# Ren-Okubo/diffusion_model

Hardware: AMD Instinct MI355X
Metric: atoms*denoise-steps/sec, 64-atom SiO2 T=1000 (higher is better)
Workload: dtype bf16; 1 GPU; 64-atom SiO2 cells x 256 graphs/GPU, 4-layer EGNN (H=36, W=1024, m=256), T=1000 reverse steps, fully connected (E=1032192/GPU); global_batch=256, parallelism=replicas x1 (no data-path collective)

## Files before the change

diffusion_model_amd/_lib.py:

```python
import ctypes as C
import os

_HERE = os.path.dirname(os.path.abspath(__file__))
LIB_PATH = os.environ.get("EGNN_LIB", os.path.join(_HERE, "libegnn_amd.so"))

PREC_F32, PREC_BF16, PREC_BF16X3, PREC_F16, PREC_F16C8 = 0, 1, 2, 3, 4
NORM_CALL, NORM_GRAPH = 0, 1
PRECISIONS = {"fp32": PREC_F32, "f32": PREC_F32, "float32": PREC_F32, "bf16": PREC_BF16, "bfloat16": PREC_BF16,
              "bf16x3": PREC_BF16X3, "f16c8": PREC_F16C8, "fp16": PREC_F16, "f16": PREC_F16, "float16": PREC_F16}
NORM_SCOPES = {"call": NORM_CALL, "graph": NORM_GRAPH}
OPTIM_ADAM, OPTIM_ADAMW_AMSGRAD, OPTIM_RADAM_SF = 0, 1, 2
KABSCH_CENTERS = {"centroid": 0, "first": 1}
KABSCH_FLIPS = {"row": 0, "column": 1}
ASSIGN_MAX_ATOMS = 1024
STRUCT_MAX_TYPES, STRUCT_MAX_ATOMS = 4, 32768
STRUCT_CENTRE_BLOCK, STRUCT_CHUNK, STRUCT_BOND_CENTRES = 64, 1024, 8
CELL_MAX_TYPES, CELL_MAX_SHELLS, CELL_MAX_ENV_ATOMS, CELL_SHIFT_CODES = 4, 4, 1024, 729
TOPO_MAX_ATOMS, TOPO_MAX_DEGREE, TOPO_BRANCH_MODULUS, TOPO_MAX_LENGTH = 1024, 32, 7, 64
RING_MAX_SITES, RING_MAX_SIZE = 4096, 32
SOAP_MAX_TYPES, SOAP_MAX_N, SOAP_MAX_L, SOAP_MAX_K = 4, 16, 10, 8
SQ_MAX_TYPES, SQ_MAX_Q, SQ_MAX_BINS, SQ_MAX_ATOMS, SQ_MAX_VECTORS = 4, 4096, 4096, 32768, 1 << 24
SQ_ROW_BLOCK, SQ_CHUNK, SQ_VECTOR_BLOCK = 64, 256, 256
SQ_WINDOWS = {None: 0, "none": 0, "lorch": 1}
CELL_CENTRE_BLOCK = 64
PREALIGN_MIN_ATOMS = 5


_FLAGS_FALLBACK = b"FLAGS := --offload-arch=gfx950 -O3 -std=c++17 -fPIC -ffp-contract=off -fno-slp-vectorize -fvisibility=hidden"


def _flags_line() -> bytes:
    try:
        with open(os.path.join(os.path.dirname(_HERE), "Makefile"), "rb") as f:
            flags = [l for l in f.read().splitlines() if l.startswith(b"FLAGS")]
        return b"\n".join(flags)
    except OSError:
        return _FLAGS_FALLBACK


def _sources_sha256(names) -> str:
    import hashlib
    h = hashlib.sha256()
    csrc = os.path.join(_HERE, "csrc")
    for name in names:
        with open(os.path.join(csrc, name), "rb") as f:
            h.update(name.encode() + b"\0" + f.read())
    h.update(_flags_line())
    return h.hexdigest()


def edge_kernel_sources_sha256() -> str:
    return _sources_sha256(("edge_x_m16.hip", "edge_bf16_v4.hip", "pack.hip", "edge_tile.h", "kernels.h", "common.h", "layer_pack.h",
                            "diag.h"))


def forward_sources_sha256() -> str:
    return _sources_sha256(("egnn_forward.hip", "host_logic.h", "host_logic.cpp", "pack.hip", "edge_x_m16.hip", "edge_bf16_v4.hip", "edge_bf16_v3.hip", "edge_small.hip",
                            "edge_bf16x3.hip", "edge_f16c8w.hip", "edge_f16c8w_mphase2.inc", "edge_f16c8w_mphasek.inc", "node_bf16.hip",
                            "edge_tile.h", "kernels.h", "common.h", "layer_pack.h", "diag.h"))


def training_sources_sha256() -> str:
    import glob
    import hashlib
    h = hashlib.sha256()
    csrc = os.path.join(_HERE, "csrc")
    names = sorted(glob.glob(os.path.join(csrc, "*.hip")) + glob.glob(os.path.join(csrc, "*.h")) + glob.glob(os.path.join(csrc, "*.cpp")) +
                   glob.glob(os.path.join(csrc, "*.inc")))
    names += [os.path.join(_HERE, "autograd.py"), os.path.join(_HERE, "gemm.py")]
    for path in names:
        with open(path, "rb") as f:
            h.update(os.path.basename(path).encode() + b"\0" + f.read())
    h.update(_flags_line())
    return h.hexdigest()


_vp, _i, _f, _u64 = C.c_void_p, C.c_int, C.c_float, C.c_uint64
_fp = C.POINTER(C.c_float)


class OptimConsts(C.Structure):
    _fields_ = [(name, C.c_float) for name in ("beta2", "one_minus_beta2", "eps", "weight_decay", "one_minus_beta1",
                                               "bias_correction2_sqrt", "step_size", "decay_mul", "bias_correction2", "ckp1",
                                               "adaptive_y_lr", "lr")] + [("rectified", C.c_int32)]


_pp, _i64p, _dp = C.POINTER(C.c_void_p), C.POINTER(C.c_int64), C.POINTER(C.c_double)

SIGNATURES = {
    "egnn_last_error": (C.c_char_p, []),
    "egnn_version": (_i, []),
    "egnn_create": (_i, [C.POINTER(_vp), _i]),
    "egnn_destroy": (_i, [_vp]),
    "egnn_set_model": (_i, [_vp] + [_i] * 6),
    "egnn_pack_layer": (_i, [_vp, _vp, _i] + [_vp] * 16),
    "egnn_set_graph": (_i, [_vp, _i, _i, _i] + [_vp] * 5),
    "egnn_set_side_stream": (_i, [_vp, _vp]),
    "egcl_forward": (_i, [_vp, _vp, _i, _i, _i] + [_vp] * 4),
    "egcl_forward_begin": (_i, [_vp, _vp, _i, _i, _i] + [_vp] * 3),
    "egcl_forward_end": (_i, [_vp, _vp, _i, _i, _i] + [_vp] * 5),
    "egnn_forward": (_i, [_vp, _vp, _i, _i] + [_vp] * 4),
    "egcl_read_aggregates": (_i, [_vp, _vp, _i] + [_vp] * 3),
    "egcl_backward_l1_act": (_i, [_vp, _i, _i, _i] + [_vp] * 7),
    "egcl_backward_heads": (_i, [_vp, _i, _i, _i, _i] + [_vp] * 20),
    "egcl_backward_l1_grad": (_i, [_vp, _i, _i, _i] + [_vp] * 7),
    "egcl_backward_gather_in": (_i, [_vp, _i, _i, _i, _i] + [_vp] * 6),
    "egcl_backward_scatter": (_i, [_vp, _i, _i, _i, _i] + [_vp] * 9),
    "egcl_backward_first_reduce": (_i, [_vp, _i, _i, _i, _i, _vp, _vp, _vp, _vp, _vp, _i, _vp, _i] + [_vp] * 9),
    "egcl_backward_node_act": (_i, [_vp, _i, _i, _vp, _i, _vp, _vp, _i, _vp, _vp, _i, _vp]),
    "egcl_backward_scatter_geom": (_i, [_vp, _i, _i] + [_vp] * 8),
    "egcl_backward_fused_supported": (_i, [_vp]),
    "egcl_backward_table": (_i, [_vp, _vp, _i, _vp]),
    "egcl_backward_edge_recompute": (_i, [_vp, _vp, _i, _vp, _vp, _vp, _i, _i] + [_vp] * 11),
    "egcl_backward_dgrad": (_i, [_vp, _vp, _i, _vp, _i, _i] + [_vp] * 4),
    "egcl_backward_dgrad_reduce": (_i, [_vp, _vp, _i, _vp, _i, _i] + [_vp] * 6),
    "egcl_forward_save": (_i, [_vp, _vp, _i, _i] + [_vp] * 9),
    "egcl_backward_heads_saved": (_i, [_vp, _vp, _i, _vp, _vp, _vp, _i, _i] + [_vp] * 10),
    "egnn_gemm_tn_workspace_bytes": (C.c_size_t, [_i, _i, _i]),
    "egnn_gemm_tn_bf16": (_i, [_vp, _i, _i, _i, _vp, _i, _vp, _i, _f, _vp, _i, _i, _i, _i, _vp, C.c_size_t]),
    "egnn_gemm_rows_pack": (_i, [_vp, _i, _i, _vp, _i, _vp]),
    "egnn_gemm_rows_bf16": (_i, [_vp, _i, _vp, _i, _i, _vp, _vp, _i, _i, _vp, _vp, _i, _i, _i]),
    "egnn_gamma_tilde": (_i, [_vp, _i, _i, _vp, _vp, _vp, _vp, _vp]),
    "egnn_dense_rows": (_i, [_vp, _i, _i, _i, _vp, _vp, _vp, _i, _vp]),
    "egnn_eps": (_i, [_vp, _i, _i, _i, _vp, _i] + [_vp] * 5),
    "egnn_remove_mean": (_i, [_vp, _i, _i, _vp, _i, _vp, _vp]),
    "schedule_table_build": (_i, [_i, C.c_double, C.c_double, _fp, _fp, _fp]),
    "schedule_table_from_alpha": (_i, [_i, _fp, _fp, _fp]),
    "ddpm_reverse_step": (_i, [_vp, _i, _i, _i, _vp, _i, _f, _f, _f, _vp, _i, _vp, _vp, _vp, _i]),
    "egnn_sampler_prepare": (_i, [_vp, _i, _i, _f, _vp, _vp, _u64]),
    "egnn_sampler_set_mode": (_i, [_vp, _i]),
    "egnn_sampler_init": (_i, [_vp, _vp, _vp, _vp]),
    "egnn_sampler_run": (_i, [_vp, _vp, _i, _i, _i, _i, _vp, _vp]),
    "egnn_sampler_final": (_i, [_vp, _vp, _i, _i] + [_vp] * 5),
    "egnn_sampler_state": (_i, [_vp, _vp, _vp, _vp, _vp, C.POINTER(_i)]),
    "ddpm_sampler_init": (_i, [_vp, _i, _i, _i, _i, _i, _vp, _vp, _f, _u64] + [_vp] * 6),
    "ddpm_sampler_step": (_i, [_vp, _i, _i, _i, _i, _i, _i, _vp, _vp, _f, _u64] + [_vp] * 7),
    "ddpm_sampler_final": (_i, [_vp, _i, _i, _i, _i, _i, _vp, _vp, _f, _u64] + [_vp] * 10),
    "egnn_fc_graph_build": (_i, [_vp, _i, _i] + [_vp] * 6),
    "egnn_radius_graph_count": (_i, [_vp, _i, _vp, _vp, _vp, _f, _vp]),
    "egnn_radius_graph_fill": (_i, [_vp, _i, _vp, _vp, _vp, _f, _vp, _vp, _vp]),
    "egnn_rdf": (_i, [_vp, _i, _vp, _vp, C.c_double, C.c_double, _f, _i, _i, _vp]),
    "egnn_si_o_si": (_i, [_vp, _i, _i, _vp, _vp, _vp, _f, _vp]),
    "egnn_kabsch": (_i, [_vp, _i, _vp, _vp, _vp, _i, _i, _vp, _vp, _i, _vp]),
    "egnn_kabsch_ordered": (_i, [_vp, _i, _vp, _vp, _vp, _vp, _i, _i, _vp]),
    "egnn_kabsch_backward": (_i, [_vp, _i, _vp, _vp, _vp, _vp, _i, _i, _vp, _vp, _vp]),
    "egnn_kabsch_grad_host": (_i, [_i, _dp, _dp, _i, _i, _dp, _dp, C.c_double, _dp, _dp]),
    "egnn_kabsch_perm_workspace_bytes": (C.c_size_t, [_i, _i]),
    "egnn_kabsch_perm": (_i, [_vp, _i, _vp, _vp, _vp, _i, _vp, _vp, _vp, _vp, _vp, C.c_size_t]),
    "egnn_assign": (_i, [_vp, _i, _vp, _vp, _vp, _i, _vp, _vp, _vp]),
    "egnn_assign_prealign": (_i, [_vp, _i, _vp, _vp, _vp, _i, _vp, _vp]),
    "egnn_struct_pair_counts": (_i, [_vp, _i, _i, _vp, _vp, _vp, _i, _vp, _i, C.c_double, _i, _vp]),
    "egnn_struct_bonds": (_i, [_vp, _i, _i, _vp, _vp, _vp, _i, _vp, _i, _f, C.c_double, _i, _vp, _vp, _vp]),
    "egnn_struct_rdf_finish": (_i, [_vp, _i, _i, _vp, _vp, _vp, C.c_double, C.c_double, C.c_double, _i, _vp]),
    "egnn_struct_counts_host": (_i, [_i, _i, _vp, _vp, _vp, C.c_double, _i, _f, C.c_double, _i, _vp, _vp, _vp, _vp]),
    "egnn_topo_bonds": (_i, [_vp, _i, _i, _i, _vp, _vp, _vp, _i, _vp, _vp, _vp, _vp, _vp]),
    "egnn_topo_paths": (_i, [_vp, _i, _i, _i, _vp, _vp, _i, _vp, _vp, _vp, _vp, _i, _vp, _vp, _vp, _vp, _vp]),
    "egnn_topo_tanimoto": (_i, [_vp, _i, _i, _vp, _i, _vp, _i, _vp, _vp, _vp, _vp]),
    "egnn_topo_host": (_i, [_i, _i, _vp, _vp, _vp, _vp, _i] + [_vp] * 8 + [_i] + [_vp] * 4),
    "egnn_rings": (_i, [_vp, _i, _vp, _i, _vp, _vp, _vp, _i, _i, _vp, _vp, _i, _i, _i] + [_vp] * 8),
    "egnn_rings_host": (_i, [_i, _vp, _i, _vp, _vp, _vp, _i, _i, _vp, _vp, _i, _i, _i] + [_vp] * 4),
    "egnn_soap_features": (_i, [_i, _i, _i]),
    "egnn_soap_table_doubles": (_i, [_i, _i]),
    "egnn_soap_descriptor": (_i, [_vp, _i, _i, _i, _vp, _vp, _vp, _i, _i, C.c_double, _vp, _i, _vp, _vp, _vp, _vp]),
    "egnn_soap_cosine": (_i, [_vp, _i, _i, _vp, _i, _vp, _i, _vp, _vp]),
    "egnn_soap_gram": (_i, [_vp, _i, _vp, _i, _vp, _i, _vp, _vp]),
    "egnn_spectrum_nearest": (_i, [_vp, _i, _i, _i, _i] + [_vp] * 6),
    "egnn_soap_host": (_i, [_i, _i, _i, _vp, _vp, _vp, _i, _i, C.c_double, _vp, _i, _vp, _vp, _vp, _i, _vp, _i, _vp, _i, _i, _vp, _vp, _vp,
                            _i, _i, _i, _i] + [_vp] * 6),
    "egnn_cell_bonds_count": (_i, [_vp, _i, _i, _vp, _vp, _vp, _vp, _vp, C.c_double, _vp, _i, _vp]),
    "egnn_cell_bonds_fill": (_i, [_vp, _i, _i, _vp, _vp, _vp, _vp, _vp, C.c_double, _vp, _i, _vp, _i, _vp, _vp]),
    "egnn_cell_env_count": (_i, [_vp, _i, _i, _vp, _vp, _vp, _i, _vp, _vp, _i, _vp, _vp, _i, _i, _vp]),
    "egnn_cell_env_fill": (_i, [_vp, _i, _i, _i, _vp, _vp, _vp, _vp, _vp, _vp, _vp, _i, _vp, _vp, _i, _vp, _vp, _i, _i, _vp, _i] + [_vp] * 4),
    "egnn_cell_env_host": (_i, [_i, _i, _vp, _vp, _vp, _vp, C.c_double, _i, _vp, _vp, _i, _i, _vp, C.c_int64, _vp, _vp, _vp, C.c_int64] + [_vp] * 4),
    "egnn_sq_debye": (_i, [_vp, _i, _i, _vp, _vp, _vp, _i, _i, _vp, _vp, C.c_double, _i, _vp, _i, _vp, _vp, _vp]),
    "egnn_sq_cell_plan": (_i, [_i, _vp, C.c_double, _vp, _vp]),
    "egnn_sq_cell_count": (_i, [_vp, _i, _vp, _vp, _vp, _vp, C.c_double, _i, _vp]),
    "egnn_sq_cell_rho": (_i, [_vp, _i, _i, _i] + [_vp] * 10 + [C.c_double, C.c_double, _i, _i, _vp, _i, _vp, _i] + [_vp] * 4),
    "egnn_sq_cell_shells": (_i, [_vp, _i, _i, _i, _vp, _vp, _i] + [_vp] * 6),
    "egnn_sq_host": (_i, [_i, _i, _i, _vp, _vp, _vp, _i, _vp, C.c_double, _i, _vp, _i, _i, _i, _vp, _vp, _vp, _vp, C.c_double, C.c_double, _i,
                          C.c_int64] + [_vp] * 8),
    "egnn_optim_step": (_i, [_vp, _i, _i, _pp, _pp, _pp, _pp, _pp, _i64p, C.POINTER(OptimConsts)]),
    "egnn_optim_interp": (_i, [_vp, _i, _pp, _pp, _i64p, _f]),
    "egnn_optim_tensors_per_launch": (_i, []),
    "egnn_debug_stamps": (_i, [_vp, C.POINTER(C.c_uint64)]),
    "egnn_profile_enable": (_i, [_vp, _i]),
    "egnn_profile_read": (_i, [_vp, _fp, C.POINTER(_i), _fp]),
}

_lib = None


def lib():
    global _lib
    if _lib is None:
        if not os.path.exists(LIB_PATH):
            raise RuntimeError(
                f"{LIB_PATH} not found: build the HIP extension first (`make` at the repo root or "
                "`python -c 'import __graft_entry__ as g; g.build()'`). There is no CPU fallback.")
        handle = C.CDLL(LIB_PATH)
        for name, (res, args) in SIGNATURES.items():
            fn = getattr(handle, name)
            fn.restype, fn.argtypes = res, args
        _lib = handle
    return _lib


class EgnnError(RuntimeError):
    pass


def check(rc):
    if rc != 0:
# ... 17 lines not shown
```

diffusion_model_amd/csrc/edge_x_m16.hip:

```cpp
#include <cstdlib>

#include "diag.h"
#include "edge_tile.h"

namespace egnn {

namespace {

#ifdef EGNN_EXP_WGSTAMP
__device__ unsigned long long g_xwg_stamps[20000][12];
#define WG_STAMP(k) DIAG_WG_STAMP(g_xwg_stamps, 20000, k)
#define WG_STAMP_HW() DIAG_WG_STAMP_HW(g_xwg_stamps, 20000, 5)
#else
#define WG_STAMP(k)
#define WG_STAMP_HW()
#endif

using namespace tile128;
constexpr size_t kA1 = (size_t)8 * kR * 16;
__host__ __device__ constexpr size_t x16_smem_bytes(int KP) { return kOffLoop + 2 * kA1 + (size_t)KP * 4; }
static_assert(x16_smem_bytes(256) == 48192 && x16_smem_bytes(512) == 49216 && x16_smem_bytes(1024) == 51264,
              "LDS allocation of the 16x16x32 coordinate kernels");

typedef __attribute__((ext_vector_type(4))) float f32x4v;

template <bool SAVE, typename V8 = bf16x8, bool PERSIST = false>
__global__ __launch_bounds__(kTileThreads, 2) void edge_x_m16_kernel(const EdgeParams p) {
  static_assert(!(SAVE && OpTraits<V8>::f16), "the training forward keeps bf16 activations");
  static_assert(!(SAVE && PERSIST), "the persistent form is the inference kernel");
  if constexpr (OpTraits<V8>::f16) f16_saturate_mode();
  extern __shared__ __attribute__((aligned(16))) char smem[];
  const Lds L(smem);
  char* s_a1 = smem + kOffLoop;
  float* s_wd = reinterpret_cast<float*>(s_a1 + 2 * kA1);

  const int tid = threadIdx.x, lane = tid & 63;
  const int wave = __builtin_amdgcn_readfirstlane(tid >> 6);
  const int r15 = lane & 15, q4 = lane >> 4;
  const int KP = p.WxP;
  const int nsplit = p.WxP / 512;
  const int NC = KP / kChunkK, KS = KP / 32;
  const rsrc_t rs_tab = make_rsrc(p.table, diag::drop_table_loads(p.dbg) ? 0u : (unsigned)((size_t)p.N * p.TC * 2));
  const rsrc_t rs_w = make_rsrc(p.w2x, diag::drop_weight_loads(p.dbg) ? 0u : (unsigned)((size_t)p.WxP * KP * 2));
  const unsigned offP = 0u, offQ = (unsigned)p.WxP * 2u;
  const unsigned lane16 = lane * 16u;
  const int nunits = PERSIST ? ((p.E + kR - 1) / kR) * nsplit : (int)gridDim.x;
  UnitH uc0, uc1;
  V8 bq[2][4];
  int pf_d0, pf_s0, pf_d1, pf_s1, pf_d, pf_s, pf_r0, pf_r1;
  float pf_x[6];
  auto unit_of = [&](const int bv, int& tile_o, int& half_o) {
    const int jj = xcd_tile(bv, nunits);
    tile_o = jj / nsplit;
    half_o = jj - tile_o * nsplit;
  };
  auto prefetch_indices = [&](const int bv, const int tq) {
    int t, h;
    unit_of(bv, t, h);
    const int ne0 = t * kR, nnv = min(kR, p.E - ne0), br = tq >> 3;
    const bool r0 = br < nnv, r1 = br + 64 < nnv, rt = tq < nnv && tq < kR;
    pf_d0 = r0 ? p.edge_dst[ne0 + br] : 0; pf_s0 = r0 ? p.edge_src[ne0 + br] : 0;
    pf_d1 = r1 ? p.edge_dst[ne0 + br + 64] : 0; pf_s1 = r1 ? p.edge_src[ne0 + br + 64] : 0;
    pf_d = rt ? p.edge_dst[ne0 + tq] : 0; pf_s = rt ? p.edge_src[ne0 + tq] : 0;
  };
  auto prefetch_data = [&](const int bv, const int tq) {
    int t, h;
    unit_of(bv, t, h);
    const unsigned k16 = (unsigned)(tq & 7) * 16u, l16 = (unsigned)(tq & 63) * 16u;
#pragma unroll
    for (int k = 0; k < 3; ++k) { pf_x[k] = p.x[3 * pf_d + k]; pf_x[3 + k] = p.x[3 * pf_s + k]; }
    pf_r0 = p.row_ptr[pf_d]; pf_r1 = p.row_ptr[pf_d + 1];
    unith_load(uc0, rs_tab, (unsigned)pf_d0 * (unsigned)p.TC * 2u + k16, (unsigned)pf_s0 * (unsigned)p.TC * 2u + k16, offP, offQ);
    unith_load(uc1, rs_tab, (unsigned)pf_d1 * (unsigned)p.TC * 2u + k16, (unsigned)pf_s1 * (unsigned)p.TC * 2u + k16, offP, offQ);
    const unsigned nw0 = (unsigned)(h * 32 + wave * 4) * KS * 1024u;
#pragma unroll
    for (int s = 0; s < 2; ++s)
#pragma unroll
      for (int cb = 0; cb < 4; ++cb) bq[s][cb] = ldbuf_v8<V8>(rs_w, l16, nw0 + ((unsigned)cb * KS + s) * 1024u);
  };
  if constexpr (PERSIST) {
    for (int i = tid; i < KP; i += kTileThreads) s_wd[i] = p.wdx[i];
    prefetch_indices(blockIdx.x, tid);
    prefetch_data(blockIdx.x, tid);
  }
  int bv = blockIdx.x;
  do {
  const int j = xcd_tile(bv, nunits);
  const int tile = j / nsplit, half = j - tile * nsplit;
  const int e0 = tile * kR;
  const int nvalid = min(kR, p.E - e0);

  DIAG_STAMP_SETUP(p.stamps + (size_t)wave * 32 * 4);
  DIAG_STAMP(30, 0);
  WG_STAMP(0);
  int tid_p = tid;
  if constexpr (PERSIST) asm volatile("" : "+v"(tid_p));
  const int lane_p = tid_p & 63;
  if constexpr (!PERSIST) {
    prologue_rows(p, L, e0, nvalid, p.wdx, KP, s_wd, tid);
  } else {
    const int tid = tid_p;
    if (tid < kR) {
      const float dx = pf_x[0] - pf_x[3], dy = pf_x[1] - pf_x[4], dz = pf_x[2] - pf_x[5];
      L.dst[tid] = pf_d;
      L.src[tid] = pf_s;
      L.diff[tid] = dx; L.diff[kR + tid] = dy; L.diff[2 * kR + tid] = dz;
      const float nrm = sqrtf(dx * dx + dy * dy + dz * dz);
      L.d2[tid] = nrm * nrm;
      reinterpret_cast<int*>(L.gseg)[tid] = pf_r0;
      reinterpret_cast<int*>(L.gseg)[kR + tid] = pf_r1;
    }
    __syncthreads();
  }
  DIAG_STAMP(30, 1);
  WG_STAMP(1);

  const BuildRows<2> b(p, L, tid, false, diag::drop_table_loads(p.dbg) ? 0u : (unsigned)((size_t)p.N * p.TC * 2),
                       PERSIST ? pf_d0 : L.dst[tid >> 3], PERSIST ? pf_s0 : L.src[tid >> 3], PERSIST ? pf_d1 : L.dst[(tid >> 3) + 64],
                       PERSIST ? pf_s1 : L.src[(tid >> 3) + 64]);
  char* slot0 = s_a1 + (size_t)b.kg * (kR * 16) + (size_t)(b.brow ^ b.kg) * 16;
  char* slot1 = slot0 + 64 * 16;
  const unsigned lds0 = (unsigned)(size_t)(__attribute__((address_space(3))) char*)s_a1;
  const unsigned abase0 = lds0 + (unsigned)q4 * (kR * 16) + (unsigned)(r15 ^ q4) * 16u;
  const unsigned abase1 = lds0 + (unsigned)(4 + q4) * (kR * 16) + (unsigned)(r15 ^ (4 + q4)) * 16u;
  const int cb0 = half * 32 + wave * 4;
  const unsigned w0 = (unsigned)cb0 * KS * 1024u;

  f32x4v acc[8][4];
#pragma unroll
  for (int rb = 0; rb < 8; ++rb)
#pragma unroll
    for (int cb = 0; cb < 4; ++cb)
#pragma unroll
      for (int i = 0; i < 4; ++i) acc[rb][cb][i] = 0.f;

  const rsrc_t rs_s1 = make_rsrc(SAVE ? p.s1_out : nullptr, SAVE ? (unsigned)((size_t)p.E * KP * 2) : 0u);
  const unsigned vs1_0 = (unsigned)(e0 + b.brow) * (unsigned)KP * 2u + (unsigned)b.kg * 16u, vs1_1 = vs1_0 + 64u * (unsigned)KP * 2u;
  auto s1_store = [&](const V8 o0, const V8 o1, const int c) {
    if (half != 0) return;
    if constexpr (diag::kNoS1) return;
    const unsigned soff = __builtin_amdgcn_readfirstlane((unsigned)c * kChunkK * 2u);
    __builtin_amdgcn_raw_buffer_store_b128(__builtin_bit_cast(u32x4, o0), rs_s1, vs1_0, soff, 0);
    __builtin_amdgcn_raw_buffer_store_b128(__builtin_bit_cast(u32x4, o1), rs_s1, vs1_1, soff, 0);
  };
  if constexpr (!PERSIST) {
    unith_load(uc0, b.tab, b.vdst0, b.vsrc0, b.offP, b.offQ);
    unith_load(uc1, b.tab, b.vdst1, b.vsrc1, b.offP, b.offQ);
#pragma unroll
    for (int s = 0; s < 2; ++s)
#pragma unroll
      for (int cb = 0; cb < 4; ++cb) bq[s][cb] = ldbuf_v8<V8>(rs_w, lane16, w0 + ((unsigned)cb * KS + s) * 1024u);
  }
  const int S = prologue_segments<false>(p, L, e0, nvalid, tid_p, lane_p, wave);
  if constexpr (PERSIST) {
    if (tid_p < S) {
      const int* rp = reinterpret_cast<const int*>(L.gseg);
      const int r0 = L.seg_rs[tid_p];
      const bool first = (e0 + r0) == rp[r0], last = (e0 + L.seg_re[tid_p] + 1) == rp[kR + r0];
      L.seg_mode[tid_p] = (first && last) ? 2 : (first ? 1 : 0);
    }
  }
  {
    const V8 o0 = unith_finish<V8>(uc0, s_wd + b.kg * 8, b.d2r0, slot0);
    const V8 o1 = unith_finish<V8>(uc1, s_wd + b.kg * 8, b.d2r1, slot1);
    if constexpr (SAVE) s1_store(o0, o1, 0);
  }
  __syncthreads();

  auto mphase = [&](const int c, const bool last) {
    const unsigned boff = (unsigned)(c & 1) * (unsigned)kA1;
    const unsigned ab0 = abase0 + boff, ab1 = abase1 + boff;
    V8 a[3];
    TILE_LDS_RD(a[0], ab0, 0); TILE_LDS_RD(a[1], ab0, 256); TILE_LDS_RD(a[2], ab0, 512);
#pragma unroll
    for (int s = 0; s < 2; ++s) {
#pragma unroll
      for (int rb = 0; rb < 8; ++rb) {
        const int u = 8 * s + rb;
        if (u <= 13) TILE_LDS_WAIT(2);
        else if (u == 14) TILE_LDS_WAIT(1);
        else TILE_LDS_WAIT(0);
        asm volatile("" : "+v"(a[u % 3]));
#pragma unroll
        for (int cb = 0; cb < 4; ++cb)
          acc[rb][cb] = mfma16(a[u % 3], bq[s][cb], acc[rb][cb]);
#ifdef XM16_PIN
        __builtin_amdgcn_sched_barrier(0);
#endif
        if (u == 0) TILE_LDS_RD(a[0], ab0, 768); if (u == 1) TILE_LDS_RD(a[1], ab0, 1024); if (u == 2) TILE_LDS_RD(a[2], ab0, 1280);
        if (u == 3) TILE_LDS_RD(a[0], ab0, 1536); if (u == 4) TILE_LDS_RD(a[1], ab0, 1792); if (u == 5) TILE_LDS_RD(a[2], ab1, 0);
        if (u == 6) TILE_LDS_RD(a[0], ab1, 256); if (u == 7) TILE_LDS_RD(a[1], ab1, 512); if (u == 8) TILE_LDS_RD(a[2], ab1, 768);
        if (u == 9) TILE_LDS_RD(a[0], ab1, 1024); if (u == 10) TILE_LDS_RD(a[1], ab1, 1280); if (u == 11) TILE_LDS_RD(a[2], ab1, 1536);
        if (u == 12) TILE_LDS_RD(a[0], ab1, 1792);
      }
      if (!last) {
        const unsigned ksn = (unsigned)((c + 1) * 2 + s) * 1024u;
#pragma unroll
        for (int cb = 0; cb < 4; ++cb) bq[s][cb] = ldbuf_v8<V8>(rs_w, lane16, w0 + (unsigned)cb * KS * 1024u + ksn);
      }
    }
  };
  UnitH ua0, ua1;
  auto vload = [&](const int cq) {
    const int c = cq < NC ? cq : NC - 1;
    const unsigned kb = (unsigned)c * kChunkK * 2u;
    unith_load(ua0, b.tab, b.vdst0, b.vsrc0, b.offP + kb, b.offQ + kb);
    unith_load(ua1, b.tab, b.vdst1, b.vsrc1, b.offP + kb, b.offQ + kb);
  };
  auto vfinish = [&](const int c) {
    const size_t nbuf = (size_t)(c & 1) * kA1;
    __builtin_amdgcn_s_setprio(3);
    const V8 o0 = unith_finish<V8>(ua0, s_wd + c * kChunkK + b.kg * 8, b.d2r0, slot0 + nbuf);
    const V8 o1 = unith_finish<V8>(ua1, s_wd + c * kChunkK + b.kg * 8, b.d2r1, slot1 + nbuf);
    __builtin_amdgcn_s_setprio(0);
    if constexpr (SAVE) s1_store(o0, o1, c);
  };
  DIAG_STAMP(30, 2);
  WG_STAMP(2);
  DIAG_RSTAMP(31, 1);
  vload(1);
  if (wave < 4) {
    const int my_mode = (!PERSIST && tid_p < S) ? segment_mode(p, L, e0, tid_p) : 0;
    for (int i = 0; i < NC - 1; ++i) {
      mphase(i, false);
      if (!PERSIST && i == 0 && tid_p < S) L.seg_mode[tid_p] = my_mode;
      vfinish(i + 1);
      vload(i + 2);
      __syncthreads();
    }
  } else {
    for (int i = 0; i < NC - 1; ++i) {
      vfinish(i + 1);
      vload(i + 2);
      __builtin_amdgcn_sched_barrier(0);
      mphase(i, false);
      __syncthreads();
    }
  }
  mphase(NC - 1, true);
  __syncthreads();
  DIAG_STAMP(30, 3);
  WG_STAMP(3);
  DIAG_RSTAMP(31, 2);

  int tid_e = tid;
  if constexpr (PERSIST) asm volatile("" : "+v"(tid_e));
  const int lane_e = tid_e & 63, r15_e = lane_e & 15, q4_e = lane_e >> 4;
  const bool more = PERSIST && bv + (int)gridDim.x < nunits;
  const int bnext = more ? bv + (int)gridDim.x : bv;
  if constexpr (PERSIST) prefetch_indices(bnext, tid_e);
  float part[32];
#pragma unroll
  for (int v = 0; v < 32; ++v) part[v] = 0.f;
  if constexpr (SAVE && !diag::kNoStage) {
#pragma unroll
    for (int cb = 0; cb < 4; ++cb) {
      const float bb = p.b2x[16 * (cb0 + cb) + r15_e];
#pragma unroll
      for (int rb = 0; rb < 8; ++rb)
#pragma unroll
        for (int i = 0; i < 4; ++i) acc[rb][cb][i] = fmaf(acc[rb][cb][i], kNegLog2e, bb);
    }
    typedef __attribute__((ext_vector_type(2))) unsigned u32x2s;
    char* tile = s_a1 + (size_t)wave * (64 * 32);
    const unsigned tile_lds = (unsigned)(size_t)(__attribute__((address_space(3))) char*)tile;
    const int g16 = lane_e >> 4, j16 = lane_e & 15;
    const unsigned rd_addr = tile_lds + (unsigned)((8 * g16 + (j16 >> 2)) * 32 + (j16 & 3) * 8);
    __bf16* tout = static_cast<__bf16*>(p.g_a2_out) + (size_t)e0 * p.WxP + 16 * cb0;
#pragma unroll
    for (int rb = 0; rb < 8; ++rb) {
#pragma unroll
      for (int cb = 0; cb < 4; ++cb) {
        u32x2s w;
        asm("v_cvt_pk_bf16_f32 %0, %1, %2" : "=v"(w.x) : "v"(acc[rb][cb][0]), "v"(acc[rb][cb][1]));
        asm("v_cvt_pk_bf16_f32 %0, %1, %2" : "=v"(w.y) : "v"(acc[rb][cb][2]), "v"(acc[rb][cb][3]));
        *reinterpret_cast<u32x2s*>(tile + (16 * cb + r15_e) * 32 + q4_e * 8) = w;
      }
      __builtin_amdgcn_wave_barrier();
      u32x2s t[2][2];
      asm volatile("s_waitcnt lgkmcnt(0)\n\t"
                   "ds_read_b64_tr_b16 %0, %4 offset:0\n\t"
                   "ds_read_b64_tr_b16 %1, %4 offset:128\n\t"
                   "ds_read_b64_tr_b16 %2, %4 offset:1024\n\t"
                   "ds_read_b64_tr_b16 %3, %4 offset:1152\n\t"
                   "s_waitcnt lgkmcnt(0)"
                   : "=&v"(t[0][0]), "=&v"(t[0][1]), "=&v"(t[1][0]), "=&v"(t[1][1]) : "v"(rd_addr) : "memory");
      if (16 * rb + j16 < nvalid - (diag::kNoT2 ? 1000 : 0)) {
#pragma unroll
        for (int k = 0; k < 2; ++k) {
          const u32x4 o = {t[k][0].x, t[k][0].y, t[k][1].x, t[k][1].y};
          *reinterpret_cast<u32x4*>(tout + (size_t)(16 * rb + j16) * p.WxP + 32 * k + 8 * g16) = o;
        }
      }
      __builtin_amdgcn_wave_barrier();
    }
  }
  typedef __attribute__((ext_vector_type(2))) float f32x2;
#pragma unroll
  for (int cb = 0; cb < 4; ++cb) {
    const int n = 16 * (cb0 + cb) + r15_e;
    const float bb = p.b2x[n], w = p.w3x[n];
    constexpr float kAcc = kNegLog2e / OpTraits<V8>::wscale;
    const f32x2 bb2 = {bb, bb}, w2 = {w, w}, k2 = {kAcc, kAcc}, one2 = {1.0f, 1.0f};
#pragma unroll
    for (int rb = 0; rb < 8; ++rb)
#pragma unroll
      for (int i = 0; i < 4; i += 2) {
        const f32x2 a2 = {acc[rb][cb][i], acc[rb][cb][i + 1]};
        const f32x2 t = SAVE ? a2 : __builtin_elementwise_fma(a2, k2, bb2);
        const f32x2 e = {__builtin_amdgcn_exp2f(t.x), __builtin_amdgcn_exp2f(t.y)};
        const f32x2 d = e + one2;
        const f32x2 rr = {__builtin_amdgcn_rcpf(d.x), __builtin_amdgcn_rcpf(d.y)};
        const f32x2 sv = t * rr;
        f32x2 pp = {part[rb * 4 + i], part[rb * 4 + i + 1]};
        pp = __builtin_elementwise_fma(w2, sv, pp);
        part[rb * 4 + i] = pp.x;
        part[rb * 4 + i + 1] = pp.y;
      }
  }
  WG_STAMP(6);
  if constexpr (PERSIST) prefetch_data(bnext, tid_e);
  {
    float t0, t1;
    butterfly16(part, lane_e, t0, t1);
    const int row = 16 * (r15_e >> 1) + 4 * q4_e + 2 * (r15_e & 1);
    L.part[wave * kR + row] = t0;
    L.part[wave * kR + row + 1] = t1;
  }
  __syncthreads();
  WG_STAMP(7);
  if (tid_e < kR) {
    float v = half == 0 ? p.scal[0] : 0.f;
#pragma unroll
    for (int w = 0; w < 8; ++w) v += L.part[w * kR + tid_e];
    L.val[tid_e] = v;
    if constexpr (SAVE) { if (tid_e < nvalid && p.s_half_out) p.s_half_out[(size_t)half * p.E + e0 + tid_e] = v; }
  }
  __syncthreads();
  WG_STAMP(8);
  coordinate_segment_sums(p, L, S, tile, half, tid_e, lane_e, wave);
  DIAG_STAMP(31, 0);
  WG_STAMP(4);
  WG_STAMP_HW();
  if constexpr (!PERSIST) break;
  if (!more) break;
  bv += (int)gridDim.x;
  __syncthreads();
  } while (true);
}

}

int init_edge_x_m16_attributes() {
  EGNN_HIP(hipFuncSetAttribute(reinterpret_cast<const void*>(&edge_x_m16_kernel<false>), hipFuncAttributeMaxDynamicSharedMemorySize,
                               160 * 1024));
  EGNN_HIP(hipFuncSetAttribute(reinterpret_cast<const void*>(&edge_x_m16_kernel<true>), hipFuncAttributeMaxDynamicSharedMemorySize,
                               160 * 1024));
  EGNN_HIP(hipFuncSetAttribute(reinterpret_cast<const void*>(&edge_x_m16_kernel<false, f16x8>), hipFuncAttributeMaxDynamicSharedMemorySize,
                               160 * 1024));
  EGNN_HIP(hipFuncSetAttribute(reinterpret_cast<const void*>(&edge_x_m16_kernel<false, bf16x8, true>), hipFuncAttributeMaxDynamicSharedMemorySize,
                               160 * 1024));
  EGNN_HIP(hipFuncSetAttribute(reinterpret_cast<const void*>(&edge_x_m16_kernel<false, f16x8, true>), hipFuncAttributeMaxDynamicSharedMemorySize,
                               160 * 1024));
  return EGNN_OK;
}

bool edge_x_m16_supported(const EdgeParams& p) {
  return (p.WxP == 512 || p.WxP == 1024) && p.w2x16 != nullptr && x16_smem_bytes(p.WxP) <= 160 * 1024 &&
         (size_t)p.N * p.TC * 2 < ((size_t)1 << 32);
}

int launch_edge_x_m16(const EdgeParams& p, hipStream_t st, bool f16, XForm form, int grid) {
  const int units = (p.E + kR - 1) / kR * (p.WxP / 512);
  const size_t sm = x16_smem_bytes(p.WxP);
  EdgeParams q = p;
  q.w2x = p.w2x16;
  switch (form) {
    case XForm::kSave:
      if (f16) { set_error("edge_x_m16: the training forward runs on bf16 operands"); return EGNN_EINVAL; }
      hipLaunchKernelGGL(edge_x_m16_kernel<true>, dim3(units), dim3(kTileThreads), sm, st, q);
      break;
    case XForm::kPersistent:
      if (f16) hipLaunchKernelGGL((edge_x_m16_kernel<false, f16x8, true>), dim3(grid), dim3(kTileThreads), sm, st, q);
      else hipLaunchKernelGGL((edge_x_m16_kernel<false, bf16x8, true>), dim3(grid), dim3(kTileThreads), sm, st, q);
      break;
    case XForm::kPerUnit:
      if (f16) hipLaunchKernelGGL((edge_x_m16_kernel<false, f16x8>), dim3(units), dim3(kTileThreads), sm, st, q);
      else hipLaunchKernelGGL(edge_x_m16_kernel<false>, dim3(units), dim3(kTileThreads), sm, st, q);
      break;
  }
  EGNN_HIP(hipGetLastError());
  return EGNN_OK;
}

}

#ifdef EGNN_EXP_WGSTAMP
extern "C" int egnn_debug_xwg_stamps(unsigned long long* host_out) {
  return hipMemcpyFromSymbol(host_out, HIP_SYMBOL(egnn::g_xwg_stamps), sizeof(unsigned long long) * 20000 * 12) == hipSuccess ? 0 : -1;
}
#endif
```

diffusion_model_amd/csrc/kernels.h:

```cpp
#pragma once
#include "common.h"

namespace egnn {

typedef __attribute__((ext_vector_type(8))) __bf16 bf16x8;
typedef __attribute__((ext_vector_type(16))) float f32x16;
typedef __attribute__((ext_vector_type(4))) float f32x4;

__device__ __forceinline__ float silu_f(float v) {
  return v * __builtin_amdgcn_rcpf(1.0f + __expf(-v));
}
__device__ __forceinline__ float silu_s(float t) { return t * __builtin_amdgcn_rcpf(1.0f + __builtin_amdgcn_exp2f(t)); }
constexpr float kNegLog2e = -1.4426950408889634f;
constexpr float kNegInvLog2e = -0.6931471805599453f;
__device__ __forceinline__ float sigmoid_f(float v) { return __builtin_amdgcn_rcpf(1.0f + __expf(-v)); }

__device__ __forceinline__ int acc_row(int reg, int lane) { return (reg & 3) + 8 * (reg >> 2) + 4 * (lane >> 5); }


__device__ __forceinline__ int xcd_tile(int b, int nwg) {
  const int xcd = b & 7, q = nwg >> 3, r = nwg & 7;
  return (xcd < r ? xcd * (q + 1) : r * (q + 1) + (xcd - r) * q) + (b >> 3);
}

struct EdgeParams {
  int N, E;
  const int* edge_dst;
  const int* edge_src;
  const int* row_ptr;
  const float* x;
  const float* table;
  int TC, WxP, WmP, MP, cbx, cbm;
  const float *wdx, *wdm, *b2x, *w3x, *b2m, *wa, *scal;
  const void *w2x, *w2m;
  const void *w2x_lo, *w2m_lo;
  const void* w2x16;
  const void* w2m16;
  const void *w2x_c8, *w2m_c8;
  const int* c8_exp;
  float *agg_m, *agg_x, *part_m, *part_x;
  size_t agg_x_stride, part_x_stride;
  unsigned long long* stamps;
  int dbg;
  const float* g_sum_x;
  const float* g_sum_m;
  void* s1_out;
  void* g_a2_out;
  float* s_half_out;
  float *g_col_a, *g_col_b, *g_scalar;
};

__host__ __device__ inline size_t edge_smem_small(int R) { return (size_t)12 * R * 4; }
__host__ __device__ inline size_t edge_a1_bytes(int R) {
  const size_t bf = (size_t)8 * (R + 1) * 16, f32 = (size_t)32 * R * 4;
  return (bf > f32 ? bf : f32);
}
__host__ __device__ inline size_t edge_smem_bytes(int R, int MP) {
  return edge_smem_small(R) + 2 * edge_a1_bytes(R) + (size_t)R * (MP + 1) * 4;
}
constexpr int kPostHC = 512;
__host__ __device__ inline size_t post_smem_bytes(int K1P, int WhP) {
  const int hc = WhP < kPostHC ? WhP : kPostHC;
  size_t hs = (size_t)hc * 33 * 4, red = (size_t)4 * 16 * 64 * 4;
  return (size_t)K1P * 33 * 4 + (hs > red ? hs : red);
}


__device__ __forceinline__ float node_sq_sum(int n, const int* __restrict__ row_ptr, int R, const float* __restrict__ agg_x,
                                             const float* __restrict__ part_x) {
  const int rp0 = row_ptr[n], rp1 = row_ptr[n + 1];
  if (rp1 <= rp0) return 0.f;
  const int t0 = rp0 / R, t1 = (rp1 - 1) / R;
  if (t0 == t1) return agg_x[(size_t)n * 4 + 3];
  float v = part_x[((size_t)t0 * 2 + 1) * 4 + 3];
  for (int t = t0 + 1; t <= t1; ++t) v += part_x[((size_t)t * 2) * 4 + 3];
  return v;
}
__device__ __forceinline__ float graph_sq_sum8(int lo, int hi, int g8, const int* __restrict__ row_ptr, int R,
                                               const float* __restrict__ agg_x, const float* __restrict__ part_x) {
  int rp0[8], rp1[8];
#pragma unroll
  for (int k = 0; k < 8; ++k) {
    const int m = lo + g8 + 8 * k;
    const bool ok = m < hi;
    rp0[k] = ok ? row_ptr[m] : 0;
    rp1[k] = ok ? row_ptr[m + 1] : 0;
  }
  float s = 0.f;
#pragma unroll
  for (int k = 0; k < 8; ++k) {
    const int m = lo + g8 + 8 * k;
    float v = 0.f;
    if (rp1[k] > rp0[k]) {
      const int t0 = rp0[k] / R, t1 = (rp1[k] - 1) / R;
      if (t0 == t1) v = agg_x[(size_t)m * 4 + 3];
      else {
        v = part_x[((size_t)t0 * 2 + 1) * 4 + 3];
        for (int t = t0 + 1; t <= t1; ++t) v += part_x[((size_t)t * 2) * 4 + 3];
      }
    }
    s += v;
  }
  s += __shfl_xor(s, 1);
  s += __shfl_xor(s, 2);
  s += __shfl_xor(s, 4);
  return s;
}

typedef __attribute__((ext_vector_type(4))) unsigned int u32x4;
typedef __amdgpu_buffer_rsrc_t rsrc_t;

__device__ __forceinline__ rsrc_t make_rsrc(const void* base, unsigned bytes) {
  return __builtin_amdgcn_make_buffer_rsrc(const_cast<void*>(base), 0, bytes, 0x00020000);
}
__device__ __forceinline__ f32x4 ldbuf_f32x4(rsrc_t rs, unsigned voff, unsigned soff) {
  return __builtin_bit_cast(f32x4, __builtin_amdgcn_raw_buffer_load_b128(rs, voff, __builtin_amdgcn_readfirstlane(soff), 0));
}
__device__ __forceinline__ bf16x8 ldbuf_bf16x8(rsrc_t rs, unsigned voff, unsigned soff) {
  return __builtin_bit_cast(bf16x8, __builtin_amdgcn_raw_buffer_load_b128(rs, voff, __builtin_amdgcn_readfirstlane(soff), 0));
}

template <int CTRL>
__device__ __forceinline__ float dpp_mov(float src) {
  return __builtin_bit_cast(float, __builtin_amdgcn_update_dpp(0, __builtin_bit_cast(int, src), CTRL, 0xF, 0xF, true));
}
template <int BANK>
__device__ __forceinline__ float dpp_sel(float a, float b) {
  return __builtin_bit_cast(float, __builtin_amdgcn_update_dpp(__builtin_bit_cast(int, a), __builtin_bit_cast(int, b), 0xE4, 0xF, BANK, false));
}
__device__ __forceinline__ float butterfly32(float (&v)[32], int lane) {
#pragma unroll
  for (int q = 0; q < 16; ++q) {
    float a = v[q], b = v[q + 16];
    asm volatile("s_nop 1\n\tv_permlane16_swap_b32 %0, %1" : "+v"(a), "+v"(b));
    v[q] = a + b;
  }
#pragma unroll
  for (int q = 0; q < 8; ++q) {
    const float ta = v[q] + dpp_mov<0x128>(v[q]);
    const float tb = v[q + 8] + dpp_mov<0x128>(v[q + 8]);
    v[q] = dpp_sel<0xC>(ta, tb);
  }
#pragma unroll
  for (int q = 0; q < 4; ++q) {
    const float ta = v[q] + dpp_mov<0x141>(v[q]);
    const float tb = v[q + 4] + dpp_mov<0x141>(v[q + 4]);
    v[q] = dpp_sel<0xA>(ta, tb);
  }
  const bool b2 = (lane & 2) != 0, b1 = (lane & 1) != 0;
#pragma unroll
  for (int q = 0; q < 2; ++q) {
    const float ta = v[q] + dpp_mov<0x4E>(v[q]);
    const float tb = v[q + 2] + dpp_mov<0x4E>(v[q + 2]);
    v[q] = b2 ? tb : ta;
  }
  const float ta = v[0] + dpp_mov<0xB1>(v[0]);
  const float tb = v[1] + dpp_mov<0xB1>(v[1]);
  return b1 ? tb : ta;
}

struct Unit {
  f32x4 p0, p1, q0, q1;
};
__device__ __forceinline__ void unit_load(Unit& u, rsrc_t tab, unsigned vdst, unsigned vsrc, unsigned sP, unsigned sQ) {
  u.p0 = ldbuf_f32x4(tab, vdst, sP);
  u.p1 = ldbuf_f32x4(tab, vdst + 16, sP);
  u.q0 = ldbuf_f32x4(tab, vsrc, sQ);
  u.q1 = ldbuf_f32x4(tab, vsrc + 16, sQ);
}
__device__ __forceinline__ void unit_finish(const Unit& u, const float* wd, float d2, char* slot) {
  const f32x4 w0 = *reinterpret_cast<const f32x4*>(wd), w1 = *reinterpret_cast<const f32x4*>(wd + 4);
  bf16x8 o;
#pragma unroll
  for (int j = 0; j < 4; ++j) {
    o[j] = (__bf16)silu_s(fmaf(w0[j], d2, u.p0[j] + u.q0[j]));
    o[j + 4] = (__bf16)silu_s(fmaf(w1[j], d2, u.p1[j] + u.q1[j]));
// ... 127 lines not shown
```

Baseline: 1.675 million atoms*denoise-steps/s.

## Reuse staged A chunks across both output halves in persistent coordinate kernel

The persistent coordinate-edge kernel now walks work so that one workgroup processes both output halves of a tile back to back. The first six K-chunks of the gathered activation tile are kept in extra LDS so the second half can skip the prologue, the segment setup and re-gathering those chunks from the table. A leftover-tail schedule handles tiles that do not divide evenly across the grid. The cost is much larger LDS per workgroup (about 146 KB at width 1024), which may cut occupancy to one workgroup per CU, and the scheduling logic is more intricate.

```diff
diff --git a/diffusion_model_amd/_lib.py b/diffusion_model_amd/_lib.py
--- a/diffusion_model_amd/_lib.py
+++ b/diffusion_model_amd/_lib.py
@@ -50,14 +50,14 @@
 
 
 def edge_kernel_sources_sha256() -> str:
-    return _sources_sha256(("edge_x_m16.hip", "edge_bf16_v4.hip", "pack.hip", "edge_tile.h", "kernels.h", "common.h", "layer_pack.h",
+    return _sources_sha256(("edge_x_m16.hip", "edge_bf16_v4.hip", "pack.hip", "edge_tile.h", "kernels.h", "x_walk.h", "common.h", "layer_pack.h",
                             "diag.h"))
 
 
 def forward_sources_sha256() -> str:
     return _sources_sha256(("egnn_forward.hip", "host_logic.h", "host_logic.cpp", "pack.hip", "edge_x_m16.hip", "edge_bf16_v4.hip", "edge_bf16_v3.hip", "edge_small.hip",
                             "edge_bf16x3.hip", "edge_f16c8w.hip", "edge_f16c8w_mphase2.inc", "edge_f16c8w_mphasek.inc", "node_bf16.hip",
-                            "edge_tile.h", "kernels.h", "common.h", "layer_pack.h", "diag.h"))
+                            "edge_tile.h", "kernels.h", "x_walk.h", "common.h", "layer_pack.h", "diag.h"))
 
 
 def training_sources_sha256() -> str:
diff --git a/diffusion_model_amd/csrc/edge_x_m16.hip b/diffusion_model_amd/csrc/edge_x_m16.hip
--- a/diffusion_model_amd/csrc/edge_x_m16.hip
+++ b/diffusion_model_amd/csrc/edge_x_m16.hip
@@ -21,6 +21,10 @@
 __host__ __device__ constexpr size_t x16_smem_bytes(int KP) { return kOffLoop + 2 * kA1 + (size_t)KP * 4; }
 static_assert(x16_smem_bytes(256) == 48192 && x16_smem_bytes(512) == 49216 && x16_smem_bytes(1024) == 51264,
               "LDS allocation of the 16x16x32 coordinate kernels");
+constexpr int kKept = 6;
+__host__ __device__ constexpr size_t x16_persist_smem_bytes(int KP) { return x16_smem_bytes(KP) + (KP == 1024 ? kKept * kA1 : 0); }
+static_assert(x16_persist_smem_bytes(512) == 49216 && x16_persist_smem_bytes(1024) == 149568 && x16_persist_smem_bytes(1024) <= 160 * 1024,
+              "LDS allocation of the persistent 16x16x32 coordinate kernel");
 
 typedef __attribute__((ext_vector_type(4))) float f32x4v;
 
@@ -44,49 +48,49 @@
   const rsrc_t rs_w = make_rsrc(p.w2x, diag::drop_weight_loads(p.dbg) ? 0u : (unsigned)((size_t)p.WxP * KP * 2));
   const unsigned offP = 0u, offQ = (unsigned)p.WxP * 2u;
   const unsigned lane16 = lane * 16u;
-  const int nunits = PERSIST ? ((p.E + kR - 1) / kR) * nsplit : (int)gridDim.x;
+  const int ntiles = (p.E + kR - 1) / kR;
+  const rsrc_t rs_tab0 = make_rsrc(p.table, 0u);
   UnitH uc0, uc1;
   V8 bq[2][4];
   int pf_d0, pf_s0, pf_d1, pf_s1, pf_d, pf_s, pf_r0, pf_r1;
   float pf_x[6];
-  auto unit_of = [&](const int bv, int& tile_o, int& half_o) {
-    const int jj = xcd_tile(bv, nunits);
-    tile_o = jj / nsplit;
-    half_o = jj - tile_o * nsplit;
-  };
-  auto prefetch_indices = [&](const int bv, const int tq) {
-    int t, h;
-    unit_of(bv, t, h);
+  auto prefetch_indices = [&](const int t, const int tq) {
     const int ne0 = t * kR, nnv = min(kR, p.E - ne0), br = tq >> 3;
     const bool r0 = br < nnv, r1 = br + 64 < nnv, rt = tq < nnv && tq < kR;
     pf_d0 = r0 ? p.edge_dst[ne0 + br] : 0; pf_s0 = r0 ? p.edge_src[ne0 + br] : 0;
     pf_d1 = r1 ? p.edge_dst[ne0 + br + 64] : 0; pf_s1 = r1 ? p.edge_src[ne0 + br + 64] : 0;
     pf_d = rt ? p.edge_dst[ne0 + tq] : 0; pf_s = rt ? p.edge_src[ne0 + tq] : 0;
   };
-  auto prefetch_data = [&](const int bv, const int tq) {
-    int t, h;
-    unit_of(bv, t, h);
+  auto prefetch_data = [&](const int h, const rsrc_t tab, const int tq) {
     const unsigned k16 = (unsigned)(tq & 7) * 16u, l16 = (unsigned)(tq & 63) * 16u;
 #pragma unroll
     for (int k = 0; k < 3; ++k) { pf_x[k] = p.x[3 * pf_d + k]; pf_x[3 + k] = p.x[3 * pf_s + k]; }
     pf_r0 = p.row_ptr[pf_d]; pf_r1 = p.row_ptr[pf_d + 1];
-    unith_load(uc0, rs_tab, (unsigned)pf_d0 * (unsigned)p.TC * 2u + k16, (unsigned)pf_s0 * (unsigned)p.TC * 2u + k16, offP, offQ);
-    unith_load(uc1, rs_tab, (unsigned)pf_d1 * (unsigned)p.TC * 2u + k16, (unsigned)pf_s1 * (unsigned)p.TC * 2u + k16, offP, offQ);
+    unith_load(uc0, tab, (unsigned)pf_d0 * (unsigned)p.TC * 2u + k16, (unsigned)pf_s0 * (unsigned)p.TC * 2u + k16, offP, offQ);
+    unith_load(uc1, tab, (unsigned)pf_d1 * (unsigned)p.TC * 2u + k16, (unsigned)pf_s1 * (unsigned)p.TC * 2u + k16, offP, offQ);
     const unsigned nw0 = (unsigned)(h * 32 + wave * 4) * KS * 1024u;
 #pragma unroll
     for (int s = 0; s < 2; ++s)
 #pragma unroll
       for (int cb = 0; cb < 4; ++cb) bq[s][cb] = ldbuf_v8<V8>(rs_w, l16, nw0 + ((unsigned)cb * KS + s) * 1024u);
   };
+  XUnit cur{0, 0, false, true};
+  int kstep = 0;
   if constexpr (PERSIST) {
+    cur = x_walk(blockIdx.x, gridDim.x, ntiles, nsplit, 0);
+    if (!cur.valid) return;
     for (int i = tid; i < KP; i += kTileThreads) s_wd[i] = p.wdx[i];
-    prefetch_indices(blockIdx.x, tid);
-    prefetch_data(blockIdx.x, tid);
-  }
-  int bv = blockIdx.x;
+    prefetch_indices(cur.tile, tid);
+    prefetch_data(cur.share, rs_tab, tid);
+  }
   do {
-  const int j = xcd_tile(bv, nunits);
-  const int tile = j / nsplit, half = j - tile * nsplit;
+  const int j = PERSIST ? 0 : xcd_tile(blockIdx.x, gridDim.x);
+  const int tile = PERSIST ? cur.tile : j / nsplit, half = PERSIST ? cur.share : j - tile * nsplit;
+  const bool kept = PERSIST && cur.kept, skip = kept && half == 1;
+  const unsigned kept_off = 2u * (unsigned)kA1 + (unsigned)KP * 4u;
+  auto chunk_off = [&](const int c) -> unsigned {
+    return (kept && c < kKept) ? kept_off + (unsigned)c * (unsigned)kA1 : (unsigned)(c & 1) * (unsigned)kA1;
+  };
   const int e0 = tile * kR;
   const int nvalid = min(kR, p.E - e0);
 
@@ -98,7 +102,7 @@
   const int lane_p = tid_p & 63;
   if constexpr (!PERSIST) {
     prologue_rows(p, L, e0, nvalid, p.wdx, KP, s_wd, tid);
-  } else {
+  } else if (!skip) {
     const int tid = tid_p;
     if (tid < kR) {
       const float dx = pf_x[0] - pf_x[3], dy = pf_x[1] - pf_x[4], dz = pf_x[2] - pf_x[5];
@@ -151,24 +155,26 @@
 #pragma unroll
       for (int cb = 0; cb < 4; ++cb) bq[s][cb] = ldbuf_v8<V8>(rs_w, lane16, w0 + ((unsigned)cb * KS + s) * 1024u);
   }
-  const int S = prologue_segments<false>(p, L, e0, nvalid, tid_p, lane_p, wave);
+  int S;
+  if (!skip) S = prologue_segments<false>(p, L, e0, nvalid, tid_p, lane_p, wave);
+  else S = L.misc[0];
   if constexpr (PERSIST) {
-    if (tid_p < S) {
+    if (!skip && tid_p < S) {
       const int* rp = reinterpret_cast<const int*>(L.gseg);
       const int r0 = L.seg_rs[tid_p];
       const bool first = (e0 + r0) == rp[r0], last = (e0 + L.seg_re[tid_p] + 1) == rp[kR + r0];
       L.seg_mode[tid_p] = (first && last) ? 2 : (first ? 1 : 0);
     }
   }
-  {
-    const V8 o0 = unith_finish<V8>(uc0, s_wd + b.kg * 8, b.d2r0, slot0);
-    const V8 o1 = unith_finish<V8>(uc1, s_wd + b.kg * 8, b.d2r1, slot1);
+  if (!skip) {
+    const V8 o0 = unith_finish<V8>(uc0, s_wd + b.kg * 8, b.d2r0, slot0 + chunk_off(0));
+    const V8 o1 = unith_finish<V8>(uc1, s_wd + b.kg * 8, b.d2r1, slot1 + chunk_off(0));
     if constexpr (SAVE) s1_store(o0, o1, 0);
   }
   __syncthreads();
 
   auto mphase = [&](const int c, const bool last) {
-    const unsigned boff = (unsigned)(c & 1) * (unsigned)kA1;
+    const unsigned boff = chunk_off(c);
     const unsigned ab0 = abase0 + boff, ab1 = abase1 + boff;
     V8 a[3];
     TILE_LDS_RD(a[0], ab0, 0); TILE_LDS_RD(a[1], ab0, 256); TILE_LDS_RD(a[2], ab0, 512);
@@ -208,7 +214,7 @@
     unith_load(ua1, b.tab, b.vdst1, b.vsrc1, b.offP + kb, b.offQ + kb);
   };
   auto vfinish = [&](const int c) {
-    const size_t nbuf = (size_t)(c & 1) * kA1;
+    const size_t nbuf = chunk_off(c);
     __builtin_amdgcn_s_setprio(3);
     const V8 o0 = unith_finish<V8>(ua0, s_wd + c * kChunkK + b.kg * 8, b.d2r0, slot0 + nbuf);
     const V8 o1 = unith_finish<V8>(ua1, s_wd + c * kChunkK + b.kg * 8, b.d2r1, slot1 + nbuf);
@@ -218,10 +224,12 @@
   DIAG_STAMP(30, 2);
   WG_STAMP(2);
   DIAG_RSTAMP(31, 1);
-  vload(1);
+  const int istart = skip ? kKept - 1 : 0;
   if (wave < 4) {
     const int my_mode = (!PERSIST && tid_p < S) ? segment_mode(p, L, e0, tid_p) : 0;
-    for (int i = 0; i < NC - 1; ++i) {
+    if constexpr (PERSIST) for (int i = 0; i < istart; ++i) mphase(i, false);
+    vload(istart + 1);
+    for (int i = istart; i < NC - 1; ++i) {
       mphase(i, false);
       if (!PERSIST && i == 0 && tid_p < S) L.seg_mode[tid_p] = my_mode;
       vfinish(i + 1);
@@ -229,7 +237,10 @@
       __syncthreads();
     }
   } else {
-    for (int i = 0; i < NC - 1; ++i) {
+    if constexpr (PERSIST) for (int i = 0; i < istart - 1; ++i) mphase(i, false);
+    vload(istart + 1);
+    if constexpr (PERSIST) { if (skip) mphase(istart - 1, false); }
+    for (int i = istart; i < NC - 1; ++i) {
       vfinish(i + 1);
       vload(i + 2);
       __builtin_amdgcn_sched_barrier(0);
@@ -246,9 +257,14 @@
   int tid_e = tid;
   if constexpr (PERSIST) asm volatile("" : "+v"(tid_e));
   const int lane_e = tid_e & 63, r15_e = lane_e & 15, q4_e = lane_e >> 4;
-  const bool more = PERSIST && bv + (int)gridDim.x < nunits;
-  const int bnext = more ? bv + (int)gridDim.x : bv;
-  if constexpr (PERSIST) prefetch_indices(bnext, tid_e);
+  XUnit nxt = cur;
+  bool more = false;
+  if constexpr (PERSIST) {
+    const XUnit n2 = x_walk(blockIdx.x, gridDim.x, ntiles, nsplit, kstep + 1);
+    more = n2.valid;
+    if (more) nxt = n2;
+    prefetch_indices(nxt.tile, tid_e);
+  }
   float part[32];
 #pragma unroll
   for (int v = 0; v < 32; ++v) part[v] = 0.f;
@@ -319,7 +335,7 @@
       }
   }
   WG_STAMP(6);
-  if constexpr (PERSIST) prefetch_data(bnext, tid_e);
+  if constexpr (PERSIST) prefetch_data(nxt.share, more && nxt.kept && nxt.share == 1 ? rs_tab0 : rs_tab, tid_e);
   {
     float t0, t1;
     butterfly16(part, lane_e, t0, t1);
@@ -344,7 +360,8 @@
   WG_STAMP_HW();
   if constexpr (!PERSIST) break;
   if (!more) break;
-  bv += (int)gridDim.x;
+  cur = nxt;
+  ++kstep;
   __syncthreads();
   } while (true);
 }
@@ -366,13 +383,13 @@
 }
 
 bool edge_x_m16_supported(const EdgeParams& p) {
-  return (p.WxP == 512 || p.WxP == 1024) && p.w2x16 != nullptr && x16_smem_bytes(p.WxP) <= 160 * 1024 &&
+  return (p.WxP == 512 || p.WxP == 1024) && p.w2x16 != nullptr && x16_persist_smem_bytes(p.WxP) <= 160 * 1024 &&
          (size_t)p.N * p.TC * 2 < ((size_t)1 << 32);
 }
 
 int launch_edge_x_m16(const EdgeParams& p, hipStream_t st, bool f16, XForm form, int grid) {
   const int units = (p.E + kR - 1) / kR * (p.WxP / 512);
-  const size_t sm = x16_smem_bytes(p.WxP);
+  const size_t sm = x16_smem_bytes(p.WxP), smp = x16_persist_smem_bytes(p.WxP);
   EdgeParams q = p;
   q.w2x = p.w2x16;
   switch (form) {
@@ -381,8 +398,8 @@
       hipLaunchKernelGGL(edge_x_m16_kernel<true>, dim3(units), dim3(kTileThreads), sm, st, q);
       break;
     case XForm::kPersistent:
-      if (f16) hipLaunchKernelGGL((edge_x_m16_kernel<false, f16x8, true>), dim3(grid), dim3(kTileThreads), sm, st, q);
-      else hipLaunchKernelGGL((edge_x_m16_kernel<false, bf16x8, true>), dim3(grid), dim3(kTileThreads), sm, st, q);
+      if (f16) hipLaunchKernelGGL((edge_x_m16_kernel<false, f16x8, true>), dim3(grid), dim3(kTileThreads), smp, st, q);
+      else hipLaunchKernelGGL((edge_x_m16_kernel<false, bf16x8, true>), dim3(grid), dim3(kTileThreads), smp, st, q);
       break;
     case XForm::kPerUnit:
       if (f16) hipLaunchKernelGGL((edge_x_m16_kernel<false, f16x8>), dim3(units), dim3(kTileThreads), sm, st, q);
diff --git a/diffusion_model_amd/csrc/kernels.h b/diffusion_model_amd/csrc/kernels.h
--- a/diffusion_model_amd/csrc/kernels.h
+++ b/diffusion_model_amd/csrc/kernels.h
@@ -18,10 +18,10 @@
 __device__ __forceinline__ int acc_row(int reg, int lane) { return (reg & 3) + 8 * (reg >> 2) + 4 * (lane >> 5); }
 
 
-__device__ __forceinline__ int xcd_tile(int b, int nwg) {
-  const int xcd = b & 7, q = nwg >> 3, r = nwg & 7;
-  return (xcd < r ? xcd * (q + 1) : r * (q + 1) + (xcd - r) * q) + (b >> 3);
-}
+}
+#include "x_walk.h"
+namespace egnn {
+
 
 struct EdgeParams {
   int N, E;
diff --git a/diffusion_model_amd/csrc/x_walk.h b/diffusion_model_amd/csrc/x_walk.h
--- /dev/null
+++ b/diffusion_model_amd/csrc/x_walk.h
@@ -0,0 +1,43 @@
+#pragma once
+
+#if defined(__HIPCC__)
+#define EGNN_XWALK_HD __host__ __device__ __forceinline__
+#else
+#define EGNN_XWALK_HD inline
+#endif
+
+namespace egnn {
+
+EGNN_XWALK_HD int xcd_tile(int b, int nwg) {
+  const int xcd = b & 7, q = nwg >> 3, r = nwg & 7;
+  return (xcd < r ? xcd * (q + 1) : r * (q + 1) + (xcd - r) * q) + (b >> 3);
+}
+
+struct XUnit {
+  int tile, share;
+  bool kept, valid;
+};
+
+EGNN_XWALK_HD XUnit x_walk(int b, int G, int T, int nshare, int k) {
+  const int S = T / G, R = T - S * G;
+  XUnit u;
+  if (k < nshare * S) {
+    const int sweep = k / nshare;
+    u.tile = sweep * G + xcd_tile(b, G);
+    u.share = k - sweep * nshare;
+    u.kept = nshare == 2;
+    u.valid = true;
+  } else {
+    const int v0 = (k - nshare * S) * G;
+    const int left = nshare * R - v0;
+    const int n = left < G ? left : G;
+    u.valid = b < n;
+    const int v = u.valid ? v0 + xcd_tile(b, n) : 0;
+    u.tile = S * G + v / nshare;
+    u.share = v % nshare;
+    u.kept = false;
+  }
+  return u;
+}
+
+}
```

Measured after the change: 1.708 million atoms*denoise-steps/s, median of 6. 1.9% higher.
